# temex12/RobustPointClouds

Measured on AMD Instinct MI355X. Metric: adversarial-train frames/sec/GPU, SECOND KITTI-3class, at 1/2/4/8 MI355X, higher is better.
Workload: dtype bf16; 1 GPU; AdversarialVoxelNet (SECOND) KITTI 3-class, batch 6/GPU, perturber active (_epoch=3); global_batch=6, frames_per_gpu=6, dense_dtype=bf16, parallelism=dp1

## Files before the change

### include/rpc_hip.h

```cpp
#ifndef RPC_HIP_H
#define RPC_HIP_H

#include <stddef.h>
#include <stdint.h>

#ifdef __cplusplus
extern "C" {
#endif

enum {
  RPC_OK = 0,
  RPC_ERR_ARG = 1,
  RPC_ERR_WORKSPACE = 2,
  RPC_ERR_UNSUPPORTED = 3,
  RPC_ERR_HIP = 4
};

const char* rpc_version(void);

size_t rpc_hard_voxelize_workspace_size(int total_points, int batch);
int rpc_hard_voxelize(const float* points, int num_features, int total_points,
                      const int* frame_offsets, int batch,
                      const float* voxel_size , const float* coors_range ,
                      int max_points, int max_voxels,
// ... 179 lines not shown
  const float* W;
  const float* gamma;
  const float* beta;
  const void* btd;
  float* dW;
  float* dgamma;
  float* dbeta;
  int h_fmt;
  unsigned* fin_ticket;
} RpcSparseLayer;
int rpc_stream_create(int which, void** out);
int rpc_stream_priority_range(int* least, int* greatest);

size_t rpc_sparse_backward_workspace_size(const RpcSparseLayer* layers, int nlayers);
int rpc_sparse_backward(const RpcSparseLayer* layers, int nlayers, const void* grad_dense, const int* coors_last,
                        const int* shape , int flags, float* dfeat ,
                        void* workspace, size_t workspace_bytes, void* stream, void* wgrad_stream);


#define RPC_DMAP_S1 0
#define RPC_DMAP_S2 1
#define RPC_DMAP_D2 2
#define RPC_DMAP_P1 3
#define RPC_DMAP_U2 4
#define RPC_DMAP_G2 5
int rpc_dense_conv(int map, const void* src, int src_pitch, int cin, const void* wt, int cout, void* out,
                   int out_pitch, int out_offset, int accumulate, float* part, const int* row_img,
                   const int* src_img, const int* out_img, void* stream);
int rpc_dense_conv_blocks(int map, const int* row_img);
int rpc_dense_conv_part_rows(int map, int cout, const int* row_img);
int rpc_dense_conv_bnbwd(const void* src, int src_pitch, int cin, const void* wt, int cout, void* out,
                         int out_pitch, const void* bnz, const float* bnp, float* part, const int* row_img,
                         void* stream);
int rpc_dense_conv_s1_kernel(int map, int cout, const int* row_img);
int rpc_dense_tune(int knob, int value);
size_t rpc_dense_wgrad_workspace_size(int map, const int* row_img, int ci, int co);
int rpc_dense_wgrad(int map, int kind, const void* x, int x_pitch, int ci, const void* dz, int dz_pitch, int co,
                    const int* row_img, const int* src_img, const int* out_img, float* dW, void* workspace,
                    size_t workspace_bytes, void* stream);
int rpc_dense_bn_apply(const void* z, int m, int c, const float* bn, void* out, int out_pitch, int out_offset,
                       void* stream);
int rpc_dense_bnbwd_blocks(int m);
int rpc_dense_bnbwd_stats(const void* dh, int dh_pitch, int dh_offset, const void* z, int m, int c,
                          const float* bn, float* part, void* stream);
int rpc_dense_bnbwd_apply(const void* dh, int dh_pitch, int dh_offset, const void* z, int m, int c,
                          const float* bn, const float* bnb, void* dz, void* stream);
int rpc_dense_wprep(const float* W, int kind, int ci, int co, int taps, int flip, void* w_fwd, void* w_dgrad,
                    void* stream);
typedef struct {
  const float* W;
  void* w_fwd;
  void* w_dgrad;
  int kind, ci, co, taps, flip;
  int co_src;
} RpcDenseWprep;
int rpc_dense_wprep_batch(const RpcDenseWprep* descs, int n, void* stream);

int rpc_dense_conv_f32(int map, const float* src, int src_pitch, int cin, const float* wt, int cout, float* out,
                       int out_pitch, int out_offset, int accumulate, float* part, const int* row_img,
                       const int* src_img, const int* out_img, void* stream);
int rpc_dense_conv_blocks_f32(int map, const int* row_img);
size_t rpc_dense_wgrad_workspace_size_f32(int map, const int* row_img, int ci, int co);
int rpc_dense_wgrad_f32(int map, int kind, const float* x, int x_pitch, int ci, const float* dz, int dz_pitch, int co,
                        const int* row_img, const int* src_img, const int* out_img, float* dW, void* workspace,
                        size_t workspace_bytes, void* stream);
int rpc_dense_bn_apply_f32(const float* z, int m, int c, const float* bn, float* out, int out_pitch, int out_offset,
// ... 200 lines not shown
```

### robustpointclouds_amd/_ffi.py

```python
from __future__ import annotations

import ctypes as C
import os
import threading

import torch

_LIB_PATH = os.environ.get("RPC_HIP_LIB") or os.path.join(os.path.dirname(os.path.abspath(__file__)), "_lib",
                                                         "librpc_hip.so")
_lock = threading.Lock()
_lib = None

RPC_ERRORS = {1: "bad argument", 2: "workspace too small", 3: "unsupported width combination",
              4: "HIP runtime error"}
PERTURBER_NPARAMS = 36

vp = C.c_void_p
i32 = C.c_int
sz = C.c_size_t
fp = C.POINTER(C.c_float)
ip = C.POINTER(C.c_int)


class PerturberCfg(C.Structure):
# ... 127 lines not shown
                              vp, vp]),
    "rpc_sparse_to_dense": (i32, [vp, vp, vp, i32, i32, ip, i32, vp, vp]),
    "rpc_sparse_dense_clear": (i32, [vp, i32, i32, ip, i32, vp, vp]),
    "rpc_dense_to_sparse_grad": (i32, [vp, vp, vp, vp, i32, i32, ip, i32, vp, vp, vp]),
    "rpc_to_bf16_rows": (i32, [vp, vp, i32, i32, i32, vp, vp]),
    "rpc_bnbwd_to_bf16_rows": (i32, [vp, vp, vp, i32, i32, vp, vp]),
    "rpc_spconv_bf16_weight_elems": (sz, [i32, i32, i32, i32]),
    "rpc_spconv_prep_weight_bf16": (i32, [vp, i32, i32, i32, i32, vp, vp]),
    "rpc_spconv_prep_weight_bf16_batch": (i32, [vp, i32, vp]),
    "rpc_spconv_gemm_bf16": (i32, [vp, i32, vp, i32, i32, i32, vp, i32, vp, vp, vp, vp, i32, vp]),
    "rpc_spconv_gemm_bf16_n": (i32, [vp, i32, i32, vp, i32, i32, i32, vp, i32, vp, vp, vp, vp, i32, vp]),
    "rpc_spconv_gemm_h16": (i32, [vp, i32, i32, i32, vp, i32, i32, i32, vp, i32, vp, vp, vp, vp, i32, vp]),
    "rpc_bn_fold_batch": (i32, [vp, i32, vp]),
    "rpc_spconv_gemm_h16_infer": (i32, [vp, i32, i32, i32, vp, i32, i32, vp, i32, vp, vp, vp, vp, vp]),
    "rpc_to_h16_rows": (i32, [vp, vp, i32, i32, i32, i32, vp, vp, vp]),
    "rpc_spconv_wgrad_h16": (i32, [vp, i32, i32, vp, i32, i32, vp, i32, vp, vp, sz, vp]),
    "rpc_sparse_res_forward_h16": (i32, [vp, vp, vp, i32, i32, vp, vp, i32, vp, vp]),
    "rpc_bn_fin_groups": (i32, [i32]),
    "rpc_bn_fin_tickets": (i32, [i32]),
    "rpc_spconv_gemm_bf16_fin": (i32, [vp, i32, i32, vp, i32, i32, i32, vp, i32, vp, vp, vp, vp, i32,
                                       C.POINTER(RpcBnFin), vp]),
    "rpc_sparse_tune": (i32, [i32, i32]),
    "rpc_spconv_gemm_res": (i32, [vp, i32, i32, vp, i32, i32, i32, vp, i32, vp, vp, vp, vp, vp, vp,
                                  C.POINTER(RpcBnFin), vp]),
    "rpc_spconv_wgrad_bf16_workspace_size": (sz, [i32, i32, i32, i32]),
    "rpc_spconv_wgrad_bf16": (i32, [vp, i32, vp, i32, i32, vp, i32, vp, vp, sz, vp]),
    "rpc_sparse_backward_workspace_size": (sz, [vp, i32]),
    "rpc_sparse_backward": (i32, [vp, i32, vp, vp, ip, i32, vp, vp, sz, vp, vp]),
    "rpc_dense_conv": (i32, [i32, vp, i32, i32, vp, i32, vp, i32, i32, i32, vp, ip, ip, ip, vp]),
    "rpc_dense_conv_blocks": (i32, [i32, ip]),
    "rpc_dense_conv_s1_kernel": (i32, [i32, i32, ip]),
    "rpc_dense_conv_part_rows": (i32, [i32, i32, ip]),
    "rpc_dense_conv_bnbwd": (i32, [vp, i32, i32, vp, i32, vp, i32, vp, vp, vp, ip, vp]),
    "rpc_dense_tune": (i32, [i32, i32]),
    "rpc_dense_wgrad_workspace_size": (sz, [i32, ip, i32, i32]),
    "rpc_dense_wgrad": (i32, [i32, i32, vp, i32, i32, vp, i32, i32, ip, ip, ip, vp, vp, sz, vp]),
    "rpc_dense_bn_apply": (i32, [vp, i32, i32, vp, vp, i32, i32, vp]),
    "rpc_dense_bnbwd_blocks": (i32, [i32]),
    "rpc_dense_bnbwd_stats": (i32, [vp, i32, i32, vp, i32, i32, vp, vp, vp]),
    "rpc_dense_bnbwd_apply": (i32, [vp, i32, i32, vp, i32, i32, vp, vp, vp, vp]),
    "rpc_dense_wprep": (i32, [vp, i32, i32, i32, i32, i32, vp, vp, vp]),
    "rpc_dense_wprep_batch": (i32, [vp, i32, vp]),
    "rpc_dense_conv_f32": (i32, [i32, vp, i32, i32, vp, i32, vp, i32, i32, i32, vp, ip, ip, ip, vp]),
    "rpc_dense_conv_blocks_f32": (i32, [i32, ip]),
    "rpc_dense_wgrad_workspace_size_f32": (sz, [i32, ip, i32, i32]),
    "rpc_dense_wgrad_f32": (i32, [i32, i32, vp, i32, i32, vp, i32, i32, ip, ip, ip, vp, vp, sz, vp]),
    "rpc_dense_bn_apply_f32": (i32, [vp, i32, i32, vp, vp, i32, i32, vp]),
    "rpc_dense_bnbwd_stats_f32": (i32, [vp, i32, i32, vp, i32, i32, vp, vp, vp]),
    "rpc_dense_bnbwd_apply_f32": (i32, [vp, i32, i32, vp, i32, i32, vp, vp, vp, vp]),
    "rpc_dense_wprep_batch_f32": (i32, [vp, i32, vp]),
    "rpc_loss_tail_forward": (i32, [vp, vp, C.c_float, vp, vp]),
    "rpc_loss_tail_backward": (i32, [vp, C.c_float, vp, vp, vp, vp]),
    "rpc_center_tail_forward": (i32, [vp, i32, vp, C.c_float, C.c_float, vp, vp]),
    "rpc_center_tail_backward": (i32, [vp, i32, C.c_float, C.c_float, vp, vp, vp, vp]),
    "rpc_clip_adamw_workspace_size": (sz, [i32]),
    "rpc_clip_adamw": (i32, [vp, vp, vp, vp, vp, vp, vp, vp, i32, i32, vp, C.POINTER(RpcAdamWHyper), C.c_float, vp,
                             vp, sz, vp]),
    "rpc_strong_perturb_workspace_size": (sz, []),
    "rpc_strong_perturb_forward": (i32, [C.POINTER(RpcStrongCfg), vp, vp, vp, C.c_longlong, vp, vp, vp, vp, vp, sz,
                                         vp]),
    "rpc_strong_perturb_backward": (i32, [vp, C.c_longlong, vp, vp, vp, vp, vp, vp]),
    "rpc_augment_points_workspace_size": (sz, [i32, i32]),
    "rpc_augment_points": (i32, [vp, i32, i32, vp, i32, vp, fp, i32, C.c_ulonglong, vp, vp, vp, sz, vp]),
    "rpc_augment_boxes": (i32, [vp, vp, i32, i32, vp, fp, vp]),
    "rpc_head_pack": (i32, [vp, i32, i32, vp, vp, i32, i32, C.c_longlong, vp]),
    "rpc_head_unpack_workspace_size": (sz, []),
# ... 119 lines not shown
```

### robustpointclouds_amd/anchor_head.py

```python
from __future__ import annotations

import ctypes as C
import math

import numpy as np
import torch
import torch.nn.functional as Fn
from torch import nn

from . import _ffi
from .base_model import det3d_gt

P1 = 3
HEAD_PAD = 128


def limit_period(val, offset=0.5, period=math.pi):
    return val - torch.floor(val / period + offset) * period


class Anchor3DRangeGenerator:
    def __init__(self, ranges, sizes=((1.6, 3.9, 1.56),), scales=(1,), rotations=(0, 1.5707963),
                 custom_values=(), reshape_out=True, size_per_range=True):
        self.ranges = [list(r) for r in ranges]
# ... 58 lines not shown
        zg = zg + hg / 2
        diag = torch.sqrt(la ** 2 + wa ** 2)
        return torch.cat([(xg - xa) / diag, (yg - ya) / diag, (zg - za) / ha, torch.log(wg / wa),
                          torch.log(lg / la), torch.log(hg / ha), rg - ra], dim=-1)

    @staticmethod
    def decode(anchors, deltas):
        xa, ya, za, wa, la, ha, ra = torch.split(anchors, 1, dim=-1)
        xt, yt, zt, wt, lt, ht, rt = torch.split(deltas, 1, dim=-1)
        za = za + ha / 2
        diag = torch.sqrt(la ** 2 + wa ** 2)
        xg, yg = xt * diag + xa, yt * diag + ya
        zg = zt * ha + za
        lg, wg, hg = torch.exp(lt) * la, torch.exp(wt) * wa, torch.exp(ht) * ha
        return torch.cat([xg, yg, zg - hg / 2, wg, lg, hg, rt + ra], dim=-1)


def anchor_table(gen: Anchor3DRangeGenerator, H: int, W: int) -> torch.Tensor:
    xs, ys, zs = [], [], []
    for rg in gen.ranges:
        r = torch.tensor(rg, dtype=torch.float32)
        xs.append(torch.linspace(r[0], r[3], W))
        ys.append(torch.linspace(r[1], r[4], H))
        zs.append(torch.linspace(r[2], r[5], 1))
    sizes = torch.tensor(gen.sizes, dtype=torch.float32).reshape(-1, 3) * gen.scales[0]
    rot = torch.tensor(gen.rotations, dtype=torch.float32)
    return torch.cat([torch.cat(xs), torch.cat(ys), torch.cat(zs), sizes.reshape(-1), rot]).contiguous()


class HeadConvFn(torch.autograd.Function):

    @staticmethod
    def forward(ctx, x, weight):
        from .dense_bev import _nhwc
        lib = _ffi.load()
        x = _nhwc(x)
        B, Cin, H, W = x.shape
        N = weight.shape[0]
        if N > HEAD_PAD or Cin % 128:
            raise RuntimeError(f"HIP head conv needs <= {HEAD_PAD} outputs and C_in % 128 == 0 (got {N}, {Cin})")
        dev = x.device
        st = _ffi.stream_of(x)
        w32 = weight.detach().reshape(N, Cin).float().contiguous()
        wf = torch.empty((1, HEAD_PAD, Cin), dtype=torch.bfloat16, device=dev)
        wd = torch.empty((1, Cin, HEAD_PAD), dtype=torch.bfloat16, device=dev)
        desc = (_ffi.RpcDenseWprep * 1)(_ffi.RpcDenseWprep(w32.data_ptr(), wf.data_ptr(), wd.data_ptr(), 0, Cin,
                                                           HEAD_PAD, 1, 0, N))
        _ffi.check(lib.rpc_dense_wprep_batch(desc, 1, st), "rpc_dense_wprep_batch(head)")
        z = torch.empty((B * H * W, HEAD_PAD), dtype=torch.bfloat16, device=dev)
        img = _ffi.int_arr((B, H, W))
        _ffi.check(lib.rpc_dense_conv(P1, _ffi.ptr(x), Cin, Cin, _ffi.ptr(wf), HEAD_PAD, _ffi.ptr(z), HEAD_PAD, 0, 0,
                                      None, img, img, img, st), "rpc_dense_conv(head)")
        ctx.save_for_backward(x, wd)
        ctx.N, ctx.wshape = N, tuple(weight.shape)
        return z

    @staticmethod
    def backward(ctx, dz):
        from .dense_bev import _image
        lib = _ffi.load()
        x, wd = ctx.saved_tensors
        B, Cin, H, W = x.shape
        dev = x.device
        dz = dz.to(torch.bfloat16).contiguous()
        st = _ffi.stream_of(dz)
        img = _ffi.int_arr((B, H, W))
        dx = None
        if ctx.needs_input_grad[0]:
            dx = _image(B, Cin, H, W, dev)
            _ffi.check(lib.rpc_dense_conv(P1, _ffi.ptr(dz), HEAD_PAD, HEAD_PAD, _ffi.ptr(wd), Cin, _ffi.ptr(dx), Cin,
                                          0, 0, None, img, img, img, st), "rpc_dense_conv(head dgrad)")
        dw = None
        if ctx.needs_input_grad[1]:
            dwp = torch.empty((HEAD_PAD, Cin, 1, 1), dtype=torch.float32, device=dev)
            wsz = lib.rpc_dense_wgrad_workspace_size(P1, img, Cin, HEAD_PAD)
            ws = _ffi.workspace(wsz, dev)
            _ffi.check(lib.rpc_dense_wgrad(P1, 0, _ffi.ptr(x), Cin, Cin, _ffi.ptr(dz), HEAD_PAD, HEAD_PAD, img, img,
                                           img, _ffi.ptr(dwp), _ffi.ptr(ws), wsz, st), "rpc_dense_wgrad(head)")
            dw = dwp[:ctx.N].reshape(ctx.wshape)
        return dx, dw


def head_pad_f32(N: int) -> int:
    return (N + 63) // 64 * 64


class HeadConvF32Fn(torch.autograd.Function):

    @staticmethod
    def forward(ctx, x, weight):
        from .dense_bev import _nhwc
        lib = _ffi.load()
        if not x.is_cuda:
            raise RuntimeError("Anchor3DHead runs on the HIP kernels only (no CPU path)")
        x = _nhwc(x, torch.float32)
        B, Cin, H, W = x.shape
        N = weight.shape[0]
        NP = head_pad_f32(N)
        if Cin % 64:
            raise RuntimeError(f"fp32 HIP head conv needs C_in % 64 == 0 (got {Cin})")
        dev = x.device
# ... 316 lines not shown
```

### robustpointclouds_amd/csrc/dense_conv.hip

```cpp
#include <hip/hip_runtime.h>
#include <stdlib.h>
#include <string.h>

#include <algorithm>

#include "common.h"
#include "dense_common.h"
#include "rpc_hip.h"

namespace rpc {
namespace dn {

constexpr int BLK = 256;
constexpr int TM = 128;
constexpr int TN = 128;
constexpr int BK = 64;
constexpr int LP = BK + 8;

typedef __bf16 bf16x8 __attribute__((ext_vector_type(8)));
typedef float f32x4 __attribute__((ext_vector_type(4)));
typedef short s16x4 __attribute__((ext_vector_type(4)));
typedef __attribute__((address_space(3))) s16x4 lds_s16x4;
typedef unsigned short u16;


__device__ __forceinline__ int d2p_tap(int j, int py, int px) {
  const int ntx = px ? 2 : 1;
  const int ty = py ? 2 * (j / ntx) : 1, tx = px ? 2 * (j % ntx) : 1;
  return ty * 3 + tx;
}

__device__ __forceinline__ u16 f2bf(float f) { return __builtin_bit_cast(u16, (__bf16)f); }
__device__ __forceinline__ float bf2f(u16 h) { return __uint_as_float((unsigned)h << 16); }

struct IG {
  const u16* src;
  int SP;
  int CIN;
  const u16* wt;
  int COUT;
  u16* out;
  int OP, OOFF;
  int accum;
  float* part;
  Img R, S, O;
  int M;
  int flat;
};

template <int MAP>
__global__ __launch_bounds__(BLK, (taps_of<MAP>() == 1 ? 4 : 2)) void k_igemm(IG g) {
  constexpr int T = taps_of<MAP>();
  constexpr int NB = T == 1 ? 1 : 2;
  constexpr int TILEB = NB * (TM + TN) * LP * 2;
  static_assert(TILEB >= TM * TN * 2, "epilogue staging");
  __shared__ __attribute__((aligned(16))) unsigned char ldsb[TILEB];
  u16 (*sX)[TM * LP] = (u16 (*)[TM * LP])ldsb;
  u16 (*sW)[TN * LP] = (u16 (*)[TN * LP])(ldsb + NB * TM * LP * 2);
  __shared__ int sRow[TM * T];
  __shared__ float sP[2][2][TN];
  const int tid = threadIdx.x, lane = tid & 63, w = tid >> 6;
  const int wc = w >> 1, wp = w & 1;
  const int ncob = g.COUT / TN, ntiles = g.flat ? gridDim.x / ncob : gridDim.x;
  int bx, cob;
  if (g.flat) {
    const int item = xcd_remap(blockIdx.x, gridDim.x);
    bx = item / ncob;
    cob = item - bx * ncob;
  } else {
    bx = xcd_remap(blockIdx.x, gridDim.x);
    cob = blockIdx.y;
  }
  const int m0 = bx * TM, n0 = cob * TN, par = MAP == M_D2P ? 3 - (int)blockIdx.z : blockIdx.z;
  const int py = par >> 1, px = par & 1;
  const int Hp = MAP == M_D2P ? (g.R.H - py + 1) >> 1 : g.R.H, Wp = MAP == M_D2P ? (g.R.W - px + 1) >> 1 : g.R.W;
  const int Mrows = MAP == M_D2P ? g.R.B * Hp * Wp : g.M;
  if (m0 >= Mrows) return;
  const int KC = g.CIN / BK, NKS = (MAP == M_D2P ? (py + 1) * (px + 1) : T) * KC;
  const u16* wbase = g.wt + (MAP == M_U2 ? (size_t)par * g.COUT * g.CIN : 0);
  const int HW = g.R.H * g.R.W;

  for (int q = tid; q < TM * T; q += BLK) {
    const int r = q / T, t = q - r * T, m = m0 + r;
    int s = -1;
    if (MAP == M_D2P) {
      if (m < Mrows && t < (py + 1) * (px + 1)) {
        const int b = m / (Hp * Wp), rem = m - b * (Hp * Wp), yy = rem / Wp, xx = rem - yy * Wp;
        s = src_row<M_D2>(b, 2 * yy + py, 2 * xx + px, d2p_tap(t, py, px), g.S);
      }
    } else if (m < g.M) {
      const int b = m / HW, rem = m - b * HW, y = rem / g.R.W, x = rem - y * g.R.W;
      s = src_row<MAP>(b, y, x, t, g.S);
    }
    sRow[q] = s;
  }
  __syncthreads();

  uint4 rx0, rx1, rx2, rx3, rw0, rw1, rw2, rw3;
  const int srow = tid >> 3, sseg = (tid & 7) * 8;
#define IG_LOAD1(S, ks)                                                                             \
  {                                                                                                 \
    const int t_ = (ks) / KC, kc_ = (ks) - t_ * KC;                                                 \
    const int sr_ = sRow[(srow + 32 * S) * T + t_];                                                 \
    const unsigned keep_ = ~(unsigned)(sr_ >> 31);                                                  \
    uint4 v_ = *(const uint4*)(g.src + (size_t)max(sr_, 0) * g.SP + kc_ * BK + sseg);                \
    rx##S = make_uint4(v_.x & keep_, v_.y & keep_, v_.z & keep_, v_.w & keep_);                     \
    const int tw_ = MAP == M_D2P ? d2p_tap(t_, py, px) : t_;                                        \
    rw##S = *(const uint4*)(wbase + ((size_t)(tw_ * g.COUT + n0 + srow + 32 * S)) * g.CIN + kc_ * BK + sseg); \
  }
#define IG_LOAD(ks) { IG_LOAD1(0, ks) IG_LOAD1(1, ks) IG_LOAD1(2, ks) IG_LOAD1(3, ks) }
#define IG_STORE1(S, buf)                                          \
  *(uint4*)&sX[buf][(srow + 32 * S) * LP + sseg] = rx##S;          \
  *(uint4*)&sW[buf][(srow + 32 * S) * LP + sseg] = rw##S;
#define IG_STORE(buf) { IG_STORE1(0, buf) IG_STORE1(1, buf) IG_STORE1(2, buf) IG_STORE1(3, buf) }

  f32x4 acc[4][4];
#pragma unroll
  for (int i = 0; i < 4; ++i)
#pragma unroll
    for (int j = 0; j < 4; ++j) acc[i][j] = (f32x4){0.f, 0.f, 0.f, 0.f};

  IG_LOAD(0)
  IG_STORE(0)
  __syncthreads();
  for (int ks = 0; ks < NKS; ++ks) {
    const int buf = NB == 2 ? (ks & 1) : 0;
    const bool more = ks + 1 < NKS;
    if (more) {
      IG_LOAD(ks + 1)
    }
    __builtin_amdgcn_sched_barrier(0);
#pragma unroll
    for (int kk = 0; kk < BK / 32; ++kk) {
      bf16x8 a[4], b[4];
#pragma unroll
      for (int i = 0; i < 4; ++i)
        a[i] = *(const bf16x8*)&sW[buf][(wc * 64 + i * 16 + (lane & 15)) * LP + kk * 32 + 8 * (lane >> 4)];
#pragma unroll
      for (int j = 0; j < 4; ++j)
        b[j] = *(const bf16x8*)&sX[buf][(wp * 64 + j * 16 + (lane & 15)) * LP + kk * 32 + 8 * (lane >> 4)];
#pragma unroll
      for (int i = 0; i < 4; ++i)
#pragma unroll
        for (int j = 0; j < 4; ++j) acc[i][j] = __builtin_amdgcn_mfma_f32_16x16x32_bf16(a[i], b[j], acc[i][j], 0, 0, 0);
    }
    if (NB == 1 && more) __syncthreads();
    if (more) {
      IG_STORE(NB == 2 ? (buf ^ 1) : 0)
    }
    __syncthreads();
  }
#undef IG_LOAD1
#undef IG_LOAD
#undef IG_STORE1
#undef IG_STORE

  if (!g.accum) {
#pragma unroll
    for (int j = 0; j < 4; ++j) {
      const int p = wp * 64 + j * 16 + (lane & 15);
#pragma unroll
      for (int i = 0; i < 4; ++i) {
        const int q4 = lane >> 4, gr = (wc * 8 + i * 2 + (q4 >> 1)) ^ (p & 15);
        const unsigned lo = (unsigned)f2bf(acc[i][j][0]) | ((unsigned)f2bf(acc[i][j][1]) << 16);
        const unsigned hi = (unsigned)f2bf(acc[i][j][2]) | ((unsigned)f2bf(acc[i][j][3]) << 16);
        *(uint2*)(ldsb + p * 256 + gr * 16 + (q4 & 1) * 8) = make_uint2(lo, hi);
      }
    }
    __syncthreads();
    const int c = tid & 15, pq = tid >> 4;
    float t1[8], t2[8];
#pragma unroll
    for (int e = 0; e < 8; ++e) t1[e] = t2[e] = 0.f;
#pragma unroll 4
    for (int k = 0; k < TM / 16; ++k) {
      const int p = pq + 16 * k, m = m0 + p;
      if (m >= Mrows) continue;
      int orow = m;
      if (MAP == M_U2) {
        const int b = m / HW, rem = m - b * HW, y = rem / g.R.W, x = rem - y * g.R.W;
        orow = out_row<MAP>(m, b, y, x, par, g.O);
      } else if (MAP == M_D2P) {
        const int b = m / (Hp * Wp), rem = m - b * (Hp * Wp), yy = rem / Wp, xx = rem - yy * Wp;
        orow = (b * g.R.H + 2 * yy + py) * g.R.W + 2 * xx + px;
      }
      const uint4 v = *(const uint4*)(ldsb + p * 256 + ((c ^ (p & 15)) * 16));
      *(uint4*)(g.out + (size_t)orow * g.OP + g.OOFF + n0 + c * 8) = v;
      const unsigned u[4] = {v.x, v.y, v.z, v.w};
#pragma unroll
// ... 2192 lines not shown
  return (unsigned)(b < 1 ? 1 : (b > 65535 ? 65535 : b));
}

static int env_int(const char* name, int dflt) {
  const char* v = getenv(name);
  return v && *v ? atoi(v) : dflt;
}
static int g_ew_var = env_int("RPC_DENSE_EW", 0);
static int g_s1_variant = env_int("RPC_DENSE_S1", 0);
static int g_wgrad_variant = env_int("RPC_DENSE_WGRAD", 0);
static int g_s1x_dbg = 0;
static int g_y_split = env_int("RPC_DENSE_YSPLIT", 1);
static int g_y_zpf = env_int("RPC_DENSE_YZPF", 1);
static int g_ig_order = 0;

static bool s1_ybig(const int* r_img, int cout) {
  const long long blocks = (long long)r_img[0] * ((r_img[1] + CT - 1) / CT) * ((r_img[2] + CT - 1) / CT) * (cout / 128);
  return blocks > 2LL * cu_count();
}
static bool s1_ytwo(const int* r_img, int cout) {
  return cout % 128 == 0 && (g_s1_variant == 4 || (g_s1_variant == 0 && s1_ybig(r_img, cout)));
}
static bool s1_small(const int* r_img, int cout) {
  const long long bx = (long long)r_img[0] * ((r_img[1] + CT - 1) / CT) * ((r_img[2] + XTW - 1) / XTW) * (cout / 128);
  return 2 * bx <= cu_count();
}
static bool s1_xwide(const int* r_img, int cout) {
  return cout % 128 == 0 && (g_s1_variant == 3 || (g_s1_variant == 0 && !s1_small(r_img, cout)));
}

static int g_s1_n32 = env_int("RPC_DENSE_S1N32", 0);
static int g_s1c_seg = env_int("RPC_DENSE_S1C_SEG", 0);
static int g_s1c_dbg = 0;

struct S1cGeo {
  int seg, nstrip, nrun, steps_per;
};
static S1cGeo s1c_geometry(const Img& R, int ci, int co, int force_seg = 0) {
  S1cGeo q;
  const int cand[3] = {96, 64, 32};
  q.seg = 96;
  int best = 1 << 30;
  for (int k = 0; k < 3; ++k) {
    const int pad = (R.W + cand[k] - 1) / cand[k] * cand[k] - R.W;
    if (pad < best) { best = pad; q.seg = cand[k]; }
  }
  if (g_s1c_seg == 32 || g_s1c_seg == 64 || g_s1c_seg == 96) q.seg = g_s1c_seg;
  if (force_seg) q.seg = force_seg;
  q.nstrip = (R.W + q.seg - 1) / q.seg;
  const int per = q.nstrip * (ci / 64) * (co / 128);
  const int nsteps = R.B * (R.H + 2);
  int nrun = cu_count() / per > 0 ? cu_count() / per : 1;
  nrun = nrun < nsteps ? nrun : nsteps;
  q.steps_per = (nsteps + nrun - 1) / nrun;
  q.nrun = (nsteps + q.steps_per - 1) / q.steps_per;
  return q;
}
static bool s1c_ok(int ci, int co) { return ci % 64 == 0 && co % 128 == 0; }

static bool s1_n32(int tiles, int cout) {
  if (g_s1_n32 == 1) return false;
  if (g_s1_n32 == 2) return true;
  return (long long)tiles * (cout / 64) < 2LL * cu_count();
}

static bool s1_wide(int tiles, int cout) {
// ... 18 lines not shown
  if (knob == 4) {
    const int old = g_s1x_dbg;
    if (value >= 0 && value <= 255) g_s1x_dbg = value;
    return old;
  }
  if (knob == 5) {
    const int old = g_s1_n32;
    if (value >= 0 && value <= 2) g_s1_n32 = value;
    return old;
  }
  if (knob == 7) {
    const int old = g_s1c_dbg;
    if (value >= 0) g_s1c_dbg = value;
    return old;
  }
  if (knob == 6) {
    const int old = g_s1c_seg;
    if (value >= 0) g_s1c_seg = value;
    return old;
  }
  if (knob == 10) {
    const int old = g_y_zpf;
    if (value == 0 || value == 1) g_y_zpf = value;
    return old;
  }
  if (knob == 8) {
    const int old = g_y_split;
    if (value == 0 || value == 1) g_y_split = value;
    return old;
  }
  if (knob == 9) {
    const int old = g_ew_var;
    if (value == 0 || value == 1) g_ew_var = value;
    return old;
  }
  if (knob == 2) {
    const int old = g_ig_order;
    if (value >= 0) g_ig_order = value;
    return old;
  }
  return RPC_ERR_ARG;
}

static int launch_s1(const IG& g, const u16* bnz, const float* bnp, hipStream_t st) {
  const int TY = (g.R.H + CT - 1) / CT, TX = (g.R.W + CT - 1) / CT;
  C3 c{g.src, g.SP, g.CIN, g.wt, g.COUT, g.out, g.OP, g.OOFF, g.accum, g.part, g.R.B, g.R.H, g.R.W, TY, TX,
       bnz, bnp, 0};
  const bool fits32 = (long long)g.M * g.SP * 2 < (1LL << 31) && 9LL * g.COUT * g.CIN * 2 < (1LL << 31);
  const int rimg[3] = {g.R.B, g.R.H, g.R.W};
  if (s1_ytwo(rimg, g.COUT) && fits32) {
    const int items = g.R.B * TY * TX * (g.COUT / 128), tail = items % cu_count();
    c.ysplit = (g_y_split && g_s1x_dbg == 0 && items > cu_count() && 2 * tail <= cu_count()) ? tail : 0;
    const dim3 grid(items + c.ysplit);
    switch (g_s1x_dbg) {
      case 1: hipLaunchKernelGGL(k_conv3x3y<1>, grid, dim3(YB), 0, st, c); break;
      case 17: hipLaunchKernelGGL(k_conv3x3y<17>, grid, dim3(YB), 0, st, c); break;
      case 64: hipLaunchKernelGGL(k_conv3x3y<64>, grid, dim3(YB), 0, st, c); break;
      case 65: hipLaunchKernelGGL(k_conv3x3y<65>, grid, dim3(YB), 0, st, c); break;
      case 81: hipLaunchKernelGGL(k_conv3x3y<81>, grid, dim3(YB), 0, st, c); break;
      case 128: hipLaunchKernelGGL(k_conv3x3y<128>, grid, dim3(YB), 0, st, c); break;
      default:
        if (bnz != nullptr && g_y_zpf) hipLaunchKernelGGL((k_conv3x3y<0, true>), grid, dim3(YB), 0, st, c);
        else hipLaunchKernelGGL(k_conv3x3y<0>, grid, dim3(YB), 0, st, c);
    }
  } else if (s1_xwide(rimg, g.COUT)) {
    if (!fits32) return RPC_ERR_UNSUPPORTED;
// ... 35 lines not shown
  g.M = g.R.B * g.R.H * g.R.W;
  g.flat = g_ig_order == 0 && cout / TN == 2;
  if (g.M == 0) return RPC_OK;
  hipStream_t st = (hipStream_t)stream;
  if (map == M_S1) return launch_s1(g, nullptr, nullptr, st);
  switch (map) {
    case M_S1: launch_igemm<M_S1>(g, 1, st); break;
    case M_S2: launch_igemm<M_S2>(g, 1, st); break;
    case M_D2:
      if (g.part) launch_igemm<M_D2>(g, 1, st);
      else launch_igemm<M_D2P>(g, 4, st);
      break;
    case M_P1: launch_igemm<M_P1>(g, 1, st); break;
    case M_U2: launch_igemm<M_U2>(g, 4, st); break;
    default: launch_igemm<M_G2>(g, 1, st); break;
  }
  RPC_LAUNCH_CHECK();
  return RPC_OK;
}

extern "C" int rpc_dense_conv_bnbwd(const void* src, int sp, int cin, const void* wt, int cout, void* out, int op,
                                    const void* bnz, const float* bnp, float* part, const int* r_img, void* stream) {
  if (!src || !wt || !out || !r_img || !bnz || !bnp || !part) return RPC_ERR_ARG;
  if (cin % BK || cout % 128 || sp < cin || op < cout || (sp & 7) || (op & 7)) return RPC_ERR_ARG;
  if (!s1_ytwo(r_img, cout) && !s1_xwide(r_img, cout)) return RPC_ERR_UNSUPPORTED;
  IG g{(const u16*)src, sp, cin, (const u16*)wt, cout, (u16*)out, op, 0, 0, part, img3(r_img), img3(r_img),
       img3(r_img), 0};
  g.M = g.R.B * g.R.H * g.R.W;
  if ((long long)g.M * g.SP * 2 >= (1LL << 31) || 9LL * g.COUT * g.CIN * 2 >= (1LL << 31)) return RPC_ERR_UNSUPPORTED;
  if (g.M == 0) return RPC_OK;
  return launch_s1(g, (const u16*)bnz, bnp, (hipStream_t)stream);
}

extern "C" int rpc_dense_conv_s1_kernel(int map, int cout, const int* r_img) {
  if (map != M_S1 || !r_img || cout % 64) return -1;
  const int TY = (r_img[1] + CT - 1) / CT, TX = (r_img[2] + CT - 1) / CT;
  if (s1_ytwo(r_img, cout)) return 3;
  if (s1_xwide(r_img, cout)) return 2;
  return s1_wide(r_img[0] * TY * TX, cout) ? 1 : 0;
}

extern "C" int rpc_dense_conv_part_rows(int map, int cout, const int* r_img) {
  if (!r_img || map < M_S1 || map > M_G2) return -1;
  if (map == M_S1 && !s1_ytwo(r_img, cout) && s1_xwide(r_img, cout))
    return r_img[0] * ((r_img[1] + CT - 1) / CT) * ((r_img[2] + XTW - 1) / XTW);
  return rpc_dense_conv_blocks(map, r_img);
}

extern "C" int rpc_dense_conv_blocks(int map, const int* r_img) {
  if (map == M_S1) return r_img[0] * ((r_img[1] + CT - 1) / CT) * ((r_img[2] + CT - 1) / CT);
  const long long M = (long long)r_img[0] * r_img[1] * r_img[2];
  return (int)((M + TM - 1) / TM) * (map == M_U2 ? 4 : 1);
}

extern "C" size_t rpc_dense_wgrad_workspace_size(int map, const int* r_img, int ci, int co) {
  const int M = r_img[0] * r_img[1] * r_img[2];
  const int T = map_wtaps(map);
  size_t n = (size_t)wgrad_chunks(M, T, ci, co);
  if (map == M_S1 && s1c_ok(ci, co)) {
    for (int seg = 32; seg <= 96; seg += 32) {
      const S1cGeo q = s1c_geometry(img3(r_img), ci, co, seg);
      const size_t c = (size_t)q.nrun * q.nstrip;
      n = c > n ? c : n;
    }
  }
  return n * T * ci * co * sizeof(float);
// ... 164 lines not shown
```

### robustpointclouds_amd/dense_bev.py

```python
from __future__ import annotations

import os
import weakref

import torch

from . import _ffi

S1, S2, D2, P1, U2, G2 = 0, 1, 2, 3, 4, 5


class ConvTimer:

    def __init__(self):
        self.recs = []
        self.enabled = False

    def start(self):
        e = torch.cuda.Event(enable_timing=True)
        e.record(torch.cuda.current_stream())
        return e

    KERNELS = {0: "rpc::dn::k_conv3x3<0>", 1: "rpc::dn::k_conv3x3w<0>", 2: "rpc::dn::k_conv3x3x<0>",
               3: "rpc::dn::k_conv3x3y<0>", 12: "rpc::dn::k_conv3x3x<0> +bnbwd", 13: "rpc::dn::k_conv3x3y<0> +bnbwd"}
# ... 259 lines not shown
        wts = _prep_weights(eng, [L], dev, st)[0]
    wf, wd = wts
    Mo = B * Ho * Wo
    z = torch.empty((Mo, L.co), dtype=eng.dt, device=dev)
    ri, si, oi = _ffi.int_arr(R), _ffi.int_arr(S), _ffi.int_arr(O)
    part = None
    if training:
        nblk = eng.part_rows(L.map, L.co, ri)
        part = torch.empty((nblk, 2 * L.co), dtype=torch.float32, device=dev)
    _ffi.check(eng.conv(L.map, _ffi.ptr(h), pitch, L.ci, _ffi.ptr(wf), L.co, _ffi.ptr(z), L.co, 0, 0,
                        _ffi.ptr(part), ri, si, oi, st), "rpc_dense_conv")
    bnm = L.bnm
    if training:
        bn = torch.empty(4 * L.co, dtype=torch.float32, device=dev)
        _ffi.check(lib.rpc_bn_finalize(_ffi.ptr(part), part.shape[0], L.co, Mo, 0, _ffi.ptr(bnm.weight),
                                       _ffi.ptr(bnm.bias), float(bnm.eps), float(bnm.momentum),
                                       _ffi.ptr(bnm.running_mean), _ffi.ptr(bnm.running_var), None, _ffi.ptr(bn),
                                       None, None, None, st), "rpc_bn_finalize")
    else:
        bn = _bn_eval(bnm, dev)
    if out is None:
        y = _image(B, L.co, Ho, Wo, dev, eng.dt)
        out_pitch, out_off = L.co, 0
    else:
        y = out
    _ffi.check(eng.bn_apply(_ffi.ptr(z), Mo, L.co, _ffi.ptr(bn), _ffi.ptr(y), out_pitch, out_off, st),
               "rpc_dense_bn_apply")
    rec = dict(L=L, h=h, pitch=pitch, z=z, bn=bn, wd=wd, R=R, S=S, O=O, in_hw=(H, W), Mo=Mo, out_bhw=(B, Ho, Wo))
    return y, rec, Ho, Wo




def _backward_layer(eng, rec, dh, dh_pitch, dh_off, dev, st, need_dx, dx_out=None, accumulate=False,
                    bn_part=None, next_rec=None):
    lib = eng.lib
    L = rec["L"]
    Mo, co, ci = rec["Mo"], L.co, L.ci
    if bn_part is not None:
        part = bn_part
        nb = part.shape[0]
    else:
        nb = lib.rpc_dense_bnbwd_blocks(Mo)
        part = torch.empty((nb, 2 * co), dtype=torch.float64 if eng.f32 else torch.float32, device=dev)
        _ffi.check(eng.bnbwd_stats(_ffi.ptr(dh), dh_pitch, dh_off, _ffi.ptr(rec["z"]), Mo, co,
                                   _ffi.ptr(rec["bn"]), _ffi.ptr(part), st), "rpc_dense_bnbwd_stats")
    bnb = torch.empty(5 * co, dtype=torch.float32, device=dev)
    dgamma = torch.empty(co, dtype=torch.float32, device=dev)
    dbeta = torch.empty(co, dtype=torch.float32, device=dev)
    mode = 1 | (4 if part.dtype == torch.float64 else 0)
    _ffi.check(lib.rpc_bn_finalize(_ffi.ptr(part), nb, co, Mo, mode, _ffi.ptr(L.bnm.weight), _ffi.ptr(L.bnm.bias),
                                   0.0, 0.0, None, None, _ffi.ptr(rec["bn"]), _ffi.ptr(bnb), _ffi.ptr(dgamma),
                                   _ffi.ptr(dbeta), None, st), "rpc_bn_finalize(bwd)")
    dz = torch.empty((Mo, co), dtype=eng.dt, device=dev)
    _ffi.check(eng.bnbwd_apply(_ffi.ptr(dh), dh_pitch, dh_off, _ffi.ptr(rec["z"]), Mo, co,
                                         _ffi.ptr(rec["bn"]), _ffi.ptr(bnb), _ffi.ptr(dz), st),
               "rpc_dense_bnbwd_apply")
    ri, si, oi = _ffi.int_arr(rec["R"]), _ffi.int_arr(rec["S"]), _ffi.int_arr(rec["O"])
    dW = torch.empty(tuple(L.conv.weight.shape), dtype=torch.float32, device=dev)
    wsz = eng.wgrad_ws(L.map, ri, ci, co)
    ws = _ffi.workspace(wsz, dev)
    _ffi.check(eng.wgrad(L.map, L.kind, _ffi.ptr(rec["h"]), rec["pitch"], ci, _ffi.ptr(dz), co, co,
                                   ri, si, oi, _ffi.ptr(dW), _ffi.ptr(ws), wsz, st), "rpc_dense_wgrad")
    dx = None
    next_part = None
    if need_dx:
        dmap = L.dgrad_map()
        B, H, W = rec["S"]
        dx = dx_out if dx_out is not None else _image(B, ci, H, W, dev, eng.dt)
        if L.map == U2:
            rd, sd = rec["R"], rec["O"]
        else:
            rd, sd = rec["S"], rec["O"]
        rc = None
        if (BN_FUSE and next_rec is not None and not eng.f32 and dmap == S1 and not accumulate and
                next_rec["L"].co == ci):
            ri_d = _ffi.int_arr(rd)
            next_part = torch.empty((lib.rpc_dense_conv_part_rows(S1, ci, ri_d), 2 * ci), dtype=torch.float32,
                                    device=dev)
            rc = _conv_bnbwd(lib, _ffi.ptr(dz), co, co, _ffi.ptr(rec["wd"]), ci, _ffi.ptr(dx), ci,
                             _ffi.ptr(next_rec["z"]), _ffi.ptr(next_rec["bn"]), _ffi.ptr(next_part), ri_d, st)
            if rc == RPC_ERR_UNSUPPORTED:
                next_part = None
            else:
                _ffi.check(rc, "rpc_dense_conv_bnbwd")
        if next_part is None:
            _ffi.check(eng.conv(dmap, _ffi.ptr(dz), co, co, _ffi.ptr(rec["wd"]), ci, _ffi.ptr(dx), ci, 0,
                                1 if accumulate else 0, None, _ffi.int_arr(rd), _ffi.int_arr(sd),
                                _ffi.int_arr(rd), st), "rpc_dense_conv(dgrad)")
    return dx, dW, dgamma, dbeta, next_part
# ... 131 lines not shown
            res = tuple(_alias(t) for t in res)
        else:
            res, _ = _backbone_bwd(eng, recs, params, need_x, gouts)
        ctx.recs = None
        ctx.eng = None
        ctx.entry = None
        return (res[0], None) + tuple(res[1:])


def _neck_fwd(eng, mod, h0, h1):
    dev = h0.device
    st = _ffi.stream_of(h0)
    layers = fpn_layers(mod)
    ins = [_nhwc(h0, eng.dt), _nhwc(h1, eng.dt)]
    B, _, H0, W0 = ins[0].shape
    Ctot = sum(L.co for L in layers)
    out = _image(B, Ctot, H0, W0, dev, eng.dt)
    recs = []
    off = 0
    wts = _prep_weights(eng, layers, dev, st)
    for L, hi, wt in zip(layers, ins, wts):
        _, C, H, W = hi.shape
        _, rec, Ho, Wo = _forward_layer(eng, L, hi, C, B, H, W, mod.training, dev, st, out=out, out_pitch=Ctot,
                                        out_off=off, wts=wt)
        assert (Ho, Wo) == (H0, W0), "FPN deblocks must upsample to the first block's resolution"
        rec["off"] = off
        recs.append(rec)
        off += L.co
    if mod.training:
        _ffi.bump_batches([L.bnm for L in layers])
    return out, (recs, Ctot)


class NeckFn(torch.autograd.Function):

    @staticmethod
    def forward(ctx, h0, h1, mod, *params):
        eng = _engine(_ffi.load(), h0)
        eng.check_widths(fpn_layers(mod))
        if GRAPHS and mod.training:
            key = ("fpn", eng.f32) + _shape_key([h0, h1]) + _state_key(mod)
            out, st_, ent = _graph_run(graph_cache(mod), key, [h0, h1], lambda a, b: _neck_fwd(eng, mod, a, b))
            out = _alias(out) if ent is not None else out
        else:
            out, st_ = _neck_fwd(eng, mod, h0, h1)
        ctx.recs, ctx.Ctot = st_
        _debug_trace(ctx.recs, mod.training)
        ctx.eng = eng
        ctx.cache = graph_cache(mod)
        ctx.param_list = params
        return out

    @staticmethod
    def backward(ctx, gout):
        eng = ctx.eng
        dev = gout.device
        st = _ffi.stream_of(gout)
        g = _nhwc(gout, eng.dt)
        grads = {}
        dins = []
        for i, rec in enumerate(ctx.recs):
            L = rec["L"]
            dx_out = None
            if GRAPHS:
                B, H, W = rec["S"]
                dx_out = _scratch_image(ctx.cache, ("fpn_dx", i, B, L.ci, H, W, eng.dt, dev), B, L.ci, H, W,
                                        dev, eng.dt)
            dx, dW, dgam, dbet, _ = _backward_layer(eng, rec, g, ctx.Ctot, rec["off"], dev, st, True, dx_out)
            grads[id(L.conv.weight)] = dW
            grads[id(L.bnm.weight)] = dgam
            grads[id(L.bnm.bias)] = dbet
            dins.append(dx)
        ctx.recs = None
        ctx.eng = None
        ctx.cache = None
        return (dins[0], dins[1], None) + tuple(grads.get(id(p)) for p in ctx.param_list)


def backbone_params(mod):
    ps = []
    for layers in second_layers(mod):
        for L in layers:
            ps += [L.conv.weight, L.bnm.weight, L.bnm.bias]
    return ps


def neck_params(mod):
    ps = []
    for L in fpn_layers(mod):
        ps += [L.conv.weight, L.bnm.weight, L.bnm.bias]
    return ps


def second_forward(mod, x):
    return BackboneFn.apply(x, mod, *backbone_params(mod))


def fpn_forward(mod, xs):
    if len(xs) != 2:
        raise RuntimeError("HIP SECONDFPN path is built for the two-block SECOND of the KITTI configs")
    return [NeckFn.apply(xs[0], xs[1], mod, *neck_params(mod))]
```

Measured before the change: 888.7 frames/s.

## Fuse head 1x1 dgrad into neck BN backward stats and apply kernels

The detection head's input-gradient 1x1 conv is no longer materialised as a separate image. Instead, the head hands its dz and weights to the neck's backward pass, which recomputes the head dgrad tile inside new implicit-GEMM kernels whose epilogues directly compute BN-backward statistics and the BN-backward apply. This removes writing and re-reading the full neck-output gradient and one kernel launch. In exchange the GEMM runs twice (once per stats pass and once for apply), the autograd plumbing returns a zero-stride placeholder gradient, and a fallback path covers unsupported shapes.

New measurement: 893.7 frames/s (median of 6 runs). Within noise of the previous version (+0.6%).

```diff
diff --git a/include/rpc_hip.h b/include/rpc_hip.h
--- a/include/rpc_hip.h
+++ b/include/rpc_hip.h
@@ -235,6 +235,12 @@
 int rpc_dense_conv_bnbwd(const void* src, int src_pitch, int cin, const void* wt, int cout, void* out,
                          int out_pitch, const void* bnz, const float* bnp, float* part, const int* row_img,
                          void* stream);
+int rpc_dense_headbn_part_rows(const int* row_img);
+int rpc_dense_headbn_stats(const void* src, int src_pitch, int k, const void* wt, int n, int c0, int c,
+                           const void* z, const float* bn, float* part, const int* row_img, void* stream);
+int rpc_dense_headbn_apply(const void* src, int src_pitch, int k, const void* wt, int n, int c0, int c,
+                           const void* z, const float* bn, const float* bnb, void* dz, const int* row_img,
+                           void* stream);
 int rpc_dense_conv_s1_kernel(int map, int cout, const int* row_img);
 int rpc_dense_tune(int knob, int value);
 size_t rpc_dense_wgrad_workspace_size(int map, const int* row_img, int ci, int co);
diff --git a/robustpointclouds_amd/_ffi.py b/robustpointclouds_amd/_ffi.py
--- a/robustpointclouds_amd/_ffi.py
+++ b/robustpointclouds_amd/_ffi.py
@@ -183,6 +183,9 @@
     "rpc_dense_conv_s1_kernel": (i32, [i32, i32, ip]),
     "rpc_dense_conv_part_rows": (i32, [i32, i32, ip]),
     "rpc_dense_conv_bnbwd": (i32, [vp, i32, i32, vp, i32, vp, i32, vp, vp, vp, ip, vp]),
+    "rpc_dense_headbn_part_rows": (i32, [ip]),
+    "rpc_dense_headbn_stats": (i32, [vp, i32, i32, vp, i32, i32, i32, vp, vp, vp, ip, vp]),
+    "rpc_dense_headbn_apply": (i32, [vp, i32, i32, vp, i32, i32, i32, vp, vp, vp, vp, ip, vp]),
     "rpc_dense_tune": (i32, [i32, i32]),
     "rpc_dense_wgrad_workspace_size": (sz, [i32, ip, i32, i32]),
     "rpc_dense_wgrad": (i32, [i32, i32, vp, i32, i32, vp, i32, i32, ip, ip, ip, vp, vp, sz, vp]),
diff --git a/robustpointclouds_amd/anchor_head.py b/robustpointclouds_amd/anchor_head.py
--- a/robustpointclouds_amd/anchor_head.py
+++ b/robustpointclouds_amd/anchor_head.py
@@ -114,9 +114,11 @@
 
     @staticmethod
     def forward(ctx, x, weight):
-        from .dense_bev import _nhwc
+        from .dense_bev import _nhwc, head_handover
         lib = _ffi.load()
+        xin = x
         x = _nhwc(x)
+        ctx.handover = head_handover(xin) if x is xin else None
         B, Cin, H, W = x.shape
         N = weight.shape[0]
         if N > HEAD_PAD or Cin % 128:
@@ -139,7 +141,7 @@
 
     @staticmethod
     def backward(ctx, dz):
-        from .dense_bev import _image
+        from .dense_bev import HeadHandover, _image
         lib = _ffi.load()
         x, wd = ctx.saved_tensors
         B, Cin, H, W = x.shape
@@ -148,7 +150,10 @@
         st = _ffi.stream_of(dz)
         img = _ffi.int_arr((B, H, W))
         dx = None
-        if ctx.needs_input_grad[0]:
+        if ctx.needs_input_grad[0] and ctx.handover is not None:
+            ctx.handover.head = (dz, wd)
+            dx = HeadHandover.zero(x.shape, dev)
+        elif ctx.needs_input_grad[0]:
             dx = _image(B, Cin, H, W, dev)
             _ffi.check(lib.rpc_dense_conv(P1, _ffi.ptr(dz), HEAD_PAD, HEAD_PAD, _ffi.ptr(wd), Cin, _ffi.ptr(dx), Cin,
                                           0, 0, None, img, img, img, st), "rpc_dense_conv(head dgrad)")
diff --git a/robustpointclouds_amd/csrc/dense_conv.hip b/robustpointclouds_amd/csrc/dense_conv.hip
--- a/robustpointclouds_amd/csrc/dense_conv.hip
+++ b/robustpointclouds_amd/csrc/dense_conv.hip
@@ -46,10 +46,138 @@
   Img R, S, O;
   int M;
   int flat;
+  const u16* bz;
+  const float* bnf;
+  const float* bnb;
+  int bstep;
 };
 
-template <int MAP>
-__global__ __launch_bounds__(BLK, (taps_of<MAP>() == 1 ? 4 : 2)) void k_igemm(IG g) {
+constexpr int EPI_STORE = 0, EPI_BNSTATS = 1, EPI_BNAPPLY = 2;
+
+__device__ __forceinline__ int bs_row(const IG& g, int b, int ps, int p) {
+  const int lg = g.COUT >> 8;
+  const int pq = p & 15, rl = pq >> lg, h = pq & ((1 << lg) - 1), k = (((ps << lg) + h) << 3) + (p >> 4);
+  const int m = b * (16 >> lg) + rl + k * g.bstep;
+  return m < g.M ? m : -1;
+}
+
+template <int EPI>
+__device__ __forceinline__ void ig_bn_epilogue(const IG& g, unsigned char* ldsb, const f32x4 (&acc)[4][4], int m0,
+                                               int n0, int bx, int ps, float (&t1)[8], float (&t2)[8]) {
+  const int tid = threadIdx.x, lane = tid & 63, w = tid >> 6, wc = w >> 1, wp = w & 1;
+  const int c = tid & 15, pq = tid >> 4, C = g.COUT, ch0 = n0 + c * 8;
+  uint4 zr[TM / 16];
+  auto row = [&](int p) { return EPI == EPI_BNSTATS ? bs_row(g, bx, ps, p) : (m0 + p < g.M ? m0 + p : -1); };
+#pragma unroll
+  for (int k = 0; k < TM / 16; ++k) zr[k] = *(const uint4*)(g.bz + (size_t)max(row(pq + 16 * k), 0) * C + ch0);
+#pragma unroll
+  for (int j = 0; j < 4; ++j) {
+    const int p = wp * 64 + j * 16 + (lane & 15);
+#pragma unroll
+    for (int i = 0; i < 4; ++i) {
+      const int q4 = lane >> 4, gr = (wc * 8 + i * 2 + (q4 >> 1)) ^ (p & 15);
+      const unsigned lo = (unsigned)f2bf(acc[i][j][0]) | ((unsigned)f2bf(acc[i][j][1]) << 16);
+      const unsigned hi = (unsigned)f2bf(acc[i][j][2]) | ((unsigned)f2bf(acc[i][j][3]) << 16);
+      *(uint2*)(ldsb + p * 256 + gr * 16 + (q4 & 1) * 8) = make_uint2(lo, hi);
+    }
+  }
+  int o0 = 0;
+  asm volatile("" : "+s"(o0));
+  const float* bnf = g.bnf + o0;
+  float sc[8], be[8], mu[8];
+#pragma unroll
+  for (int j = 0; j < 8; ++j) {
+    sc[j] = bnf[ch0 + j];
+    be[j] = bnf[C + ch0 + j];
+    mu[j] = bnf[2 * C + ch0 + j];
+  }
+  __syncthreads();
+  if (EPI == EPI_BNAPPLY) {
+    float gi[8], m1[8], m2[8], mb[8], ib[8];
+#pragma unroll
+    for (int j = 0; j < 8; ++j) {
+      gi[j] = g.bnb[ch0 + j];
+      m1[j] = g.bnb[C + ch0 + j];
+      m2[j] = g.bnb[2 * C + ch0 + j];
+      mb[j] = g.bnb[3 * C + ch0 + j];
+      ib[j] = g.bnb[4 * C + ch0 + j];
+    }
+#pragma unroll
+    for (int k = 0; k < TM / 16; ++k) {
+      const int p = pq + 16 * k, m = row(p);
+      if (m < 0) continue;
+      const uint4 v = *(const uint4*)(ldsb + p * 256 + ((c ^ (p & 15)) * 16));
+      float o[8];
+#pragma unroll
+      for (int j = 0; j < 8; ++j) {
+        const float zz = bf2f(((const u16*)&zr[k])[j]);
+        const float pre = fmaf(zz - mu[j], sc[j], be[j]);
+        const float d = pre > 0.f ? bf2f(((const u16*)&v)[j]) : 0.f;
+        const float xh = (zz - mb[j]) * ib[j];
+        o[j] = gi[j] * (d - m1[j] - xh * m2[j]);
+      }
+      u16 ob[8];
+#pragma unroll
+      for (int j = 0; j < 8; ++j) ob[j] = f2bf(o[j]);
+      *(uint4*)(g.out + (size_t)m * g.OP + g.OOFF + ch0) = *(const uint4*)ob;
+    }
+    return;
+  }
+  float is[8];
+#pragma unroll
+  for (int j = 0; j < 8; ++j) is[j] = bnf[3 * C + ch0 + j];
+  const int RL = 2048 / C, G = 16 / RL, myh = pq % G;
+  if (ps > 0 && G > 1) {
+#pragma unroll
+    for (int e = 0; e < 8; ++e) {
+      const float a1 = __shfl_down(t1[e], 16 * (G - 1), 64), a2 = __shfl_down(t2[e], 16 * (G - 1), 64);
+      if (myh == 0) { t1[e] = a1; t2[e] = a2; }
+    }
+  }
+#pragma unroll 1
+  for (int h = 0; h < G; ++h) {
+    if (h > 0) {
+#pragma unroll
+      for (int e = 0; e < 8; ++e) {
+        const float a1 = __shfl_up(t1[e], 16, 64), a2 = __shfl_up(t2[e], 16, 64);
+        if (myh == h) { t1[e] = a1; t2[e] = a2; }
+      }
+    }
+#pragma unroll
+    for (int k = 0; k < TM / 16; ++k) {
+      const int p = pq + 16 * k;
+      if (myh != h || row(p) < 0) continue;
+      const uint4 v = *(const uint4*)(ldsb + p * 256 + ((c ^ (p & 15)) * 16));
+#pragma unroll
+      for (int j = 0; j < 8; ++j) {
+        const float zz = bf2f(((const u16*)&zr[k])[j]);
+        const float pre = fmaf(zz - mu[j], sc[j], be[j]);
+        const float d = pre > 0.f ? bf2f(((const u16*)&v)[j]) : 0.f;
+        t1[j] += d;
+        t2[j] += d * ((zz - mu[j]) * is[j]);
+      }
+    }
+  }
+  __syncthreads();
+  if (ps == 0) return;
+  float* sR = (float*)ldsb;
+  if (myh == G - 1) {
+    const int rl = pq / G;
+#pragma unroll
+    for (int e = 0; e < 8; ++e) {
+      sR[(rl * 2 + 0) * TN + c * 8 + e] = t1[e];
+      sR[(rl * 2 + 1) * TN + c * 8 + e] = t2[e];
+    }
+  }
+  __syncthreads();
+  const int k2 = tid >> 7, ch = tid & 127;
+  float a = 0.f;
+  for (int r = 0; r < RL; ++r) a += sR[(r * 2 + k2) * TN + ch];
+  g.part[(size_t)bx * 2 * C + k2 * C + n0 + ch] = a;
+}
+
+template <int MAP, int EPI = EPI_STORE>
+__global__ __launch_bounds__(BLK, (taps_of<MAP>() == 1 ? (EPI == EPI_BNSTATS ? 2 : 4) : 2)) void k_igemm(IG g) {
   constexpr int T = taps_of<MAP>();
   constexpr int NB = T == 1 ? 1 : 2;
   constexpr int TILEB = NB * (TM + TN) * LP * 2;
@@ -75,15 +203,26 @@
   const int py = par >> 1, px = par & 1;
   const int Hp = MAP == M_D2P ? (g.R.H - py + 1) >> 1 : g.R.H, Wp = MAP == M_D2P ? (g.R.W - px + 1) >> 1 : g.R.W;
   const int Mrows = MAP == M_D2P ? g.R.B * Hp * Wp : g.M;
-  if (m0 >= Mrows) return;
+  if (EPI != EPI_BNSTATS && m0 >= Mrows) return;
   const int KC = g.CIN / BK, NKS = (MAP == M_D2P ? (py + 1) * (px + 1) : T) * KC;
   const u16* wbase = g.wt + (MAP == M_U2 ? (size_t)par * g.COUT * g.CIN : 0);
   const int HW = g.R.H * g.R.W;
 
+  f32x4 acc[4][4];
+  constexpr int NPASS = EPI == EPI_BNSTATS ? 2 : 1;
+  float t1[8], t2[8];
+  if constexpr (EPI == EPI_BNSTATS) {
+#pragma unroll
+    for (int e = 0; e < 8; ++e) t1[e] = t2[e] = 0.f;
+  }
+#pragma unroll 1
+  for (int ps = 0; ps < NPASS; ++ps) {
   for (int q = tid; q < TM * T; q += BLK) {
     const int r = q / T, t = q - r * T, m = m0 + r;
     int s = -1;
-    if (MAP == M_D2P) {
+    if (EPI == EPI_BNSTATS) {
+      s = bs_row(g, bx, ps, q);
+    } else if (MAP == M_D2P) {
       if (m < Mrows && t < (py + 1) * (px + 1)) {
         const int b = m / (Hp * Wp), rem = m - b * (Hp * Wp), yy = rem / Wp, xx = rem - yy * Wp;
         s = src_row<M_D2>(b, 2 * yy + py, 2 * xx + px, d2p_tap(t, py, px), g.S);
@@ -114,7 +253,6 @@
   *(uint4*)&sW[buf][(srow + 32 * S) * LP + sseg] = rw##S;
 #define IG_STORE(buf) { IG_STORE1(0, buf) IG_STORE1(1, buf) IG_STORE1(2, buf) IG_STORE1(3, buf) }
 
-  f32x4 acc[4][4];
 #pragma unroll
   for (int i = 0; i < 4; ++i)
 #pragma unroll
@@ -155,6 +293,9 @@
 #undef IG_STORE1
 #undef IG_STORE
 
+  if constexpr (EPI != EPI_STORE) ig_bn_epilogue<EPI>(g, ldsb, acc, m0, n0, bx, ps, t1, t2);
+  }
+  if constexpr (EPI != EPI_STORE) return;
   if (!g.accum) {
 #pragma unroll
     for (int j = 0; j < 4; ++j) {
@@ -2413,6 +2554,7 @@
 static int g_s1_n32 = env_int("RPC_DENSE_S1N32", 0);
 static int g_s1c_seg = env_int("RPC_DENSE_S1C_SEG", 0);
 static int g_s1c_dbg = 0;
+static int g_headfuse = env_int("RPC_DENSE_HEADFUSE", 1);
 
 struct S1cGeo {
   int seg, nstrip, nrun, steps_per;
@@ -2497,6 +2639,11 @@
   if (knob == 9) {
     const int old = g_ew_var;
     if (value == 0 || value == 1) g_ew_var = value;
+    return old;
+  }
+  if (knob == 11) {
+    const int old = g_headfuse;
+    if (value == 0 || value == 1) g_headfuse = value;
     return old;
   }
   if (knob == 2) {
@@ -2598,6 +2745,45 @@
   return launch_s1(g, (const u16*)bnz, bnp, (hipStream_t)stream);
 }
 
+static int headbn(int epi, const void* src, int sp, int k, const void* wt, int n, int c0, int c, const void* z,
+                  const float* bn, const float* bnb, float* part, void* dz, const int* r_img, void* stream) {
+  if (!src || !wt || !z || !bn || !r_img || (epi == EPI_BNSTATS ? !part : (!bnb || !dz))) return RPC_ERR_ARG;
+  const long long M = (long long)r_img[0] * r_img[1] * r_img[2];
+  if (!g_headfuse || k < BK || k % BK || (c != 128 && c != 256 && c != 512) || M > 2048LL * 256 || c0 < 0 || c0 + c > n || sp < k || (sp & 7) || M < 0 ||
+      M * sp * 2 >= (1LL << 31) || M * c * 2 >= (1LL << 31) || (long long)n * k * 2 >= (1LL << 31))
+    return RPC_ERR_UNSUPPORTED;
+  if (M == 0) return RPC_OK;
+  IG g{(const u16*)src, sp, k, (const u16*)wt + (size_t)c0 * k, c, (u16*)dz, c, 0, 0, part,
+       img3(r_img), img3(r_img), img3(r_img), (int)M, 1, (const u16*)z, bn, bnb, 0};
+  if (epi == EPI_BNSTATS) {
+    const int nb = rpc_dense_bnbwd_blocks(g.M);
+    g.bstep = nb * (2048 / c);
+    hipLaunchKernelGGL((k_igemm<M_P1, EPI_BNSTATS>), dim3(nb * (c / TN)), dim3(BLK), 0, (hipStream_t)stream, g);
+  } else {
+    hipLaunchKernelGGL((k_igemm<M_P1, EPI_BNAPPLY>), dim3(cdivu(g.M, TM) * (c / TN)), dim3(BLK), 0,
+                       (hipStream_t)stream, g);
+  }
+  RPC_LAUNCH_CHECK();
+  return RPC_OK;
+}
+
+extern "C" int rpc_dense_headbn_part_rows(const int* r_img) {
+  if (!r_img) return -1;
+  const long long M = (long long)r_img[0] * r_img[1] * r_img[2];
+  return M > 2048LL * 256 ? -1 : rpc_dense_bnbwd_blocks((int)M);
+}
+
+extern "C" int rpc_dense_headbn_stats(const void* src, int sp, int k, const void* wt, int n, int c0, int c,
+                                      const void* z, const float* bn, float* part, const int* r_img, void* stream) {
+  return headbn(EPI_BNSTATS, src, sp, k, wt, n, c0, c, z, bn, nullptr, part, nullptr, r_img, stream);
+}
+
+extern "C" int rpc_dense_headbn_apply(const void* src, int sp, int k, const void* wt, int n, int c0, int c,
+                                      const void* z, const float* bn, const float* bnb, void* dz, const int* r_img,
+                                      void* stream) {
+  return headbn(EPI_BNAPPLY, src, sp, k, wt, n, c0, c, z, bn, bnb, nullptr, dz, r_img, stream);
+}
+
 extern "C" int rpc_dense_conv_s1_kernel(int map, int cout, const int* r_img) {
   if (map != M_S1 || !r_img || cout % 64) return -1;
   const int TY = (r_img[1] + CT - 1) / CT, TX = (r_img[2] + CT - 1) / CT;
diff --git a/robustpointclouds_amd/dense_bev.py b/robustpointclouds_amd/dense_bev.py
--- a/robustpointclouds_amd/dense_bev.py
+++ b/robustpointclouds_amd/dense_bev.py
@@ -315,12 +315,34 @@
 
 
 
+def _head_dgrad(lib, head, img, dev, st, out=None):
+    dzh, wd = head
+    K, N = dzh.shape[1], wd.shape[1]
+    B, H, W = img
+    g = out if out is not None else _image(B, N, H, W, dev)
+    ri = _ffi.int_arr(img)
+    _ffi.check(lib.rpc_dense_conv(P1, _ffi.ptr(dzh), K, K, _ffi.ptr(wd), N, _ffi.ptr(g), N, 0,
+                                  0 if out is None else 1, None, ri, ri, ri, st), "rpc_dense_conv(head dgrad)")
+    return g
+
+
 def _backward_layer(eng, rec, dh, dh_pitch, dh_off, dev, st, need_dx, dx_out=None, accumulate=False,
-                    bn_part=None, next_rec=None):
+                    bn_part=None, next_rec=None, head=None):
     lib = eng.lib
     L = rec["L"]
     Mo, co, ci = rec["Mo"], L.co, L.ci
-    if bn_part is not None:
+    if head is not None:
+        dzh, hwd = head
+        hargs = (_ffi.ptr(dzh), dzh.shape[1], dzh.shape[1], _ffi.ptr(hwd), hwd.shape[1], dh_off, co,
+                 _ffi.ptr(rec["z"]), _ffi.ptr(rec["bn"]))
+        ri_h = _ffi.int_arr(rec["out_bhw"])
+        nb = lib.rpc_dense_headbn_part_rows(ri_h)
+        part = torch.empty((nb, 2 * co), dtype=torch.float32, device=dev)
+        rc = lib.rpc_dense_headbn_stats(*hargs, _ffi.ptr(part), ri_h, st)
+        if rc == RPC_ERR_UNSUPPORTED:
+            return None
+        _ffi.check(rc, "rpc_dense_headbn_stats")
+    elif bn_part is not None:
         part = bn_part
         nb = part.shape[0]
     else:
@@ -336,9 +358,13 @@
                                    0.0, 0.0, None, None, _ffi.ptr(rec["bn"]), _ffi.ptr(bnb), _ffi.ptr(dgamma),
                                    _ffi.ptr(dbeta), None, st), "rpc_bn_finalize(bwd)")
     dz = torch.empty((Mo, co), dtype=eng.dt, device=dev)
-    _ffi.check(eng.bnbwd_apply(_ffi.ptr(dh), dh_pitch, dh_off, _ffi.ptr(rec["z"]), Mo, co,
-                                         _ffi.ptr(rec["bn"]), _ffi.ptr(bnb), _ffi.ptr(dz), st),
-               "rpc_dense_bnbwd_apply")
+    if head is not None:
+        _ffi.check(lib.rpc_dense_headbn_apply(*hargs, _ffi.ptr(bnb), _ffi.ptr(dz), ri_h, st),
+                   "rpc_dense_headbn_apply")
+    else:
+        _ffi.check(eng.bnbwd_apply(_ffi.ptr(dh), dh_pitch, dh_off, _ffi.ptr(rec["z"]), Mo, co,
+                                   _ffi.ptr(rec["bn"]), _ffi.ptr(bnb), _ffi.ptr(dz), st),
+                   "rpc_dense_bnbwd_apply")
     ri, si, oi = _ffi.int_arr(rec["R"]), _ffi.int_arr(rec["S"]), _ffi.int_arr(rec["O"])
     dW = torch.empty(tuple(L.conv.weight.shape), dtype=torch.float32, device=dev)
     wsz = eng.wgrad_ws(L.map, ri, ci, co)
@@ -536,6 +562,34 @@
     return out, (recs, Ctot)
 
 
+class HeadHandover:
+    _ZERO = {}
+
+    def __init__(self):
+        self.claimed = False
+        self.head = None
+
+    @classmethod
+    def zero(cls, shape, dev):
+        z = cls._ZERO.get(dev)
+        if z is None:
+            z = cls._ZERO[dev] = torch.zeros(1, dtype=torch.bfloat16, device=dev)
+        return z.expand(shape)
+
+    @classmethod
+    def is_zero(cls, t):
+        z = cls._ZERO.get(t.device)
+        return z is not None and t.data_ptr() == z.data_ptr() and not any(t.stride())
+
+
+def head_handover(x):
+    slot = getattr(x.grad_fn, "head_slot", None)
+    if not isinstance(slot, HeadHandover) or slot.claimed or _ffi.load().rpc_dense_tune(11, -1) != 1:
+        return None
+    slot.claimed = True
+    return slot
+
+
 class NeckFn(torch.autograd.Function):
 
     @staticmethod
@@ -553,6 +607,7 @@
         ctx.eng = eng
         ctx.cache = graph_cache(mod)
         ctx.param_list = params
+        ctx.head_slot = HeadHandover() if mod.training and not eng.f32 else None
         return out
 
     @staticmethod
@@ -560,7 +615,16 @@
         eng = ctx.eng
         dev = gout.device
         st = _ffi.stream_of(gout)
-        g = _nhwc(gout, eng.dt)
+        head = None
+        if ctx.head_slot is not None:
+            head, ctx.head_slot.head = ctx.head_slot.head, None
+        g = None
+        if head is None:
+            g = _nhwc(gout, eng.dt)
+        elif not HeadHandover.is_zero(gout):
+            g = _head_dgrad(eng.lib, head, ctx.recs[0]["out_bhw"], dev, st,
+                            out=_nhwc(gout, eng.dt).clone(memory_format=torch.channels_last))
+            head = None
         grads = {}
         dins = []
         for i, rec in enumerate(ctx.recs):
@@ -570,7 +634,15 @@
                 B, H, W = rec["S"]
                 dx_out = _scratch_image(ctx.cache, ("fpn_dx", i, B, L.ci, H, W, eng.dt, dev), B, L.ci, H, W,
                                         dev, eng.dt)
-            dx, dW, dgam, dbet, _ = _backward_layer(eng, rec, g, ctx.Ctot, rec["off"], dev, st, True, dx_out)
+            res = None
+            if head is not None:
+                res = _backward_layer(eng, rec, None, ctx.Ctot, rec["off"], dev, st, True, dx_out, head=head)
+                if res is None:
+                    g = _head_dgrad(eng.lib, head, rec["out_bhw"], dev, st)
+                    head = None
+            if res is None:
+                res = _backward_layer(eng, rec, g, ctx.Ctot, rec["off"], dev, st, True, dx_out)
+            dx, dW, dgam, dbet, _ = res
             grads[id(L.conv.weight)] = dW
             grads[id(L.bnm.weight)] = dgam
             grads[id(L.bnm.bias)] = dbet
@@ -578,6 +650,7 @@
         ctx.recs = None
         ctx.eng = None
         ctx.cache = None
+        ctx.head_slot = None
         return (dins[0], dins[1], None) + tuple(grads.get(id(p)) for p in ctx.param_list)
 
 
```
